# Zanue/EndoDAV

Hardware: AMD Instinct MI355X
Metric: depth frames/sec (518x518, T=8 clip) (higher is better)
Workload: dtype f32

## Files before the change

### endodav_amd/_lib.py

```python
from __future__ import annotations

import ctypes as C
import os
from typing import Optional

_HERE = os.path.dirname(os.path.abspath(__file__))
LIB_PATH = os.environ.get("EDV_LIB_PATH") or os.path.join(_HERE, "lib", "libendodav_hip.so")
ABI_VERSION = 15

LORA_TYPES = {"none": 0, "lora": 1, "dvlora": 2, "ssb": 3, "dash": 4}
ACT_NONE, ACT_GELU, ACT_RELU, ACT_SIGMOID, ACT_SIGMOID_NEG = 0, 1, 2, 3, 4


class EdvConfig(C.Structure):

    _fields_ = [
        ("abi_version", C.c_int32),
        ("embed_dim", C.c_int32),
        ("depth", C.c_int32),
        ("num_heads", C.c_int32),
        ("taps", C.c_int32 * 4),
        ("features", C.c_int32),
        ("out_channels", C.c_int32 * 4),
        ("image_h", C.c_int32),
        ("image_w", C.c_int32),
        ("num_frames", C.c_int32),
        ("pos_tokens", C.c_int32),
        ("lora_type", C.c_int32),
        ("lora_rank", C.c_int32),
        ("include_cls_token", C.c_int32),
        ("conv_head", C.c_int32),
        ("inv_sigmoid", C.c_int32),
        ("out_sigmoid", C.c_int32),
        ("temporal_lora", C.c_int32),
        ("dash_active", C.c_int32),
        ("use_clstoken", C.c_int32),
        ("residual_mask", C.c_uint32),
        ("use_bn", C.c_int32),
        ("pe_rope", C.c_int32),
    ]


_fp = C.c_void_p
_i32, _i64, _f32, _f64 = C.c_int32, C.c_int64, C.c_float, C.c_double

SIGNATURES = {
    "edv_abi_version": (C.c_int, []),
    "edv_last_error": (C.c_char_p, []),
    "edv_create": (C.c_int, [C.POINTER(EdvConfig), C.POINTER(C.c_void_p)]),
    "edv_destroy": (C.c_int, [C.c_void_p]),
    "edv_bind_param": (C.c_int, [C.c_void_p, C.c_char_p, _fp, C.POINTER(_i64), _i32]),
    "edv_prepare": (C.c_int, [C.c_void_p, C.c_void_p]),
    "edv_refresh_lora": (C.c_int, [C.c_void_p, C.c_void_p]),
    "edv_forward": (C.c_int, [C.c_void_p, _fp, _i32, _i32, _i32, _i32, C.POINTER(C.c_void_p), C.c_void_p]),
    "edv_output_shape": (C.c_int, [C.c_void_p, _i32, C.POINTER(_i32), C.POINTER(_i32)]),
    "edv_stage_copy": (C.c_int, [C.c_void_p, C.c_char_p, _fp, C.POINTER(C.c_size_t), C.c_void_p]),
    "edv_set_capture": (C.c_int, [C.c_void_p, C.c_int]),
    "edv_profile_enable": (C.c_int, [C.c_void_p, C.c_uint32]),
    "edv_set_encoder_streams": (C.c_int, [C.c_void_p, _i32]),
    "edv_set_products": (C.c_int, [C.c_void_p, _i32, C.c_void_p]),
    "edv_get_products": (C.c_int, [C.c_void_p]),
    "edv_profile_set_mask": (C.c_int, [C.c_void_p, C.c_uint32]),
    "edv_profile_work": (C.c_int, [C.c_void_p, _i32, C.POINTER(_f64), C.POINTER(_f64)]),
    "edv_profile_read": (C.c_int, [C.c_void_p, _i32, C.POINTER(_i32), C.POINTER(_f64)]),
    "edv_device_bytes": (C.c_size_t, [C.c_void_p]),
    "edv_last_launch_count": (C.c_int, [C.c_void_p]),
    "edv_layernorm": (C.c_int, [_fp, _fp, _fp, _fp, _i64, _i32, _f32, _fp, _i32, _i32, C.c_void_p]),
    "edv_gemm_workspace": (C.c_size_t, []),
    "edv_gemm_x6_planes_bytes": (C.c_size_t, [_i32, _i32]),
    "edv_gemm_x6_split": (C.c_int, [_fp, C.c_void_p, _i32, _i32, C.c_void_p]),
    "edv_gemm_x6": (C.c_int, [_fp, C.c_void_p, _fp, _i64, _i32, _i32, _fp, _i32, _fp, _fp, _fp, C.c_size_t, C.c_void_p]),
    "edv_gemm": (C.c_int, [_fp, _fp, _fp, _i64, _i32, _i32, _fp, _i32, _fp, _fp, _fp, C.c_size_t, C.c_void_p]),
    "edv_pack_geglu": (C.c_int, [_fp, _fp, _fp, _fp, _i32, _i32, C.c_void_p]),
    "edv_gemm_geglu": (C.c_int, [_fp, _fp, _fp, _fp, _i64, _i32, _i32, C.c_void_p]),
    "edv_conv3x3": (C.c_int, [_fp, _fp, _fp, _fp, _i32, _i32, _i32, _i32, _i32, _i32, _i32, _i32, _fp, _fp, C.c_void_p]),
    "edv_conv3x3_ws": (C.c_int, [_fp, _fp, _fp, _fp, _i32, _i32, _i32, _i32, _i32, _i32, _i32, _i32, _fp, _fp, _fp, C.c_size_t, C.c_void_p]),
    "edv_set_conv_impl": (C.c_int, [_i32]),
    "edv_conv3x3_dot": (C.c_int, [_fp, _fp, _fp, _fp, _i32, _i32, _i32, _i32, _i32, _i32, _i32, _i32, _fp, _fp, _i32, C.c_void_p]),
    "edv_pack_conv3x3": (C.c_int, [_fp, _fp, _i32, _i32, C.c_void_p]),
    "edv_conv_transpose": (C.c_int, [_fp, _fp, _fp, _fp, _fp, _fp, _i32, _i32, _i32, _i32, _i32, C.c_void_p]),
    "edv_attn_spatial_workspace": (C.c_size_t, [_i32, _i32, _i32]),
    "edv_attn_spatial": (C.c_int, [_fp, _fp, _i32, _i32, _i32, _fp, C.c_size_t, _fp, C.c_void_p]),
    "edv_set_train": (C.c_int, [C.c_void_p, _i32]),
    "edv_set_grad_scope": (C.c_int, [C.c_void_p, _i32, _i32, _i32, _i32]),
    "edv_set_bias_grads": (C.c_int, [C.c_void_p, _i32, _i32]),
    "edv_generation": (C.c_int, [C.c_void_p, C.POINTER(C.c_uint64)]),
    "edv_backward": (C.c_int, [C.c_void_p, C.c_uint64, _fp, C.POINTER(C.c_void_p), C.c_void_p]),
    "edv_grad_bind_flat": (C.c_int, [C.c_void_p, _i32, C.POINTER(C.c_char_p), C.POINTER(_i64), _fp, _i64, C.POINTER(_i64)]),
    "edv_grad": (C.c_int, [C.c_void_p, C.c_char_p, C.POINTER(C.c_void_p), C.POINTER(_i64)]),
    "edv_grad_copy": (C.c_int, [C.c_void_p, C.c_char_p, _fp, _i64, C.c_void_p]),
    "edv_attn_spatial_x6_workspace": (C.c_size_t, [_i32, _i32, _i32]),
    "edv_attn_spatial_x6": (C.c_int, [_fp, _fp, _i32, _i32, _i32, _fp, C.c_size_t, C.c_void_p]),
    "edv_attn_spatial_bwd_workspace": (C.c_size_t, [_i32, _i32, _i32]),
    "edv_attn_spatial_bwd": (C.c_int, [_fp, _fp, _fp, _fp, _fp, _fp, _i32, _i32, _i32, _fp, C.c_size_t, C.c_void_p]),
    "edv_layernorm_bwd": (C.c_int, [_fp, _fp, _fp, _fp, _i64, _i32, C.c_float, _i32, C.c_void_p]),
    "edv_ew_bwd": (C.c_int, [_fp, _fp, _fp, _fp, _i64, _i32, C.c_void_p]),
    "edv_geglu_bwd": (C.c_int, [_fp, _fp, _fp, _i64, _i32, C.c_void_p]),
    "edv_transpose_scale": (C.c_int, [_fp, _fp, _fp, _i32, _i32, C.c_void_p]),
    "edv_lora_grads_workspace": (C.c_size_t, [_i64, _i32, _i32, _i32]),
    "edv_lora_grads": (C.c_int, [_fp, _fp, _i64, _i32, _i32, _i32, _fp, _fp, _fp, _fp, C.c_float, _fp, _fp, C.c_size_t, _fp, _fp, _fp, _fp, C.c_void_p]),
    "edv_bilinear_bwd": (C.c_int, [_fp, _fp, _i32, _i32, _i32, _i32, _i32, _i32, _i32, C.c_void_p]),
    "edv_dot_channels_bwd": (C.c_int, [_fp, _fp, _fp, _fp, _fp, _fp, _i64, _i32, _i32, C.c_void_p]),
    "edv_conv3x3_wgrad_workspace": (C.c_size_t, [_i32, _i32, _i32, _i32, _i32]),
    "edv_conv3x3_wgrad": (C.c_int, [_fp, _fp, _fp, _i32, _i32, _i32, _i32, _i32, _fp, C.c_size_t, _i32, C.c_void_p]),
    "edv_colsum_workspace": (C.c_size_t, [_i32]),
    "edv_colsum_rows": (C.c_int, [_fp, _fp, _i64, _i32, _fp, C.c_size_t, _fp, _i32, C.c_void_p]),
    "edv_colsum_batch_workspace": (C.c_size_t, [_i32, C.POINTER(_i64), C.POINTER(_i32)]),
    "edv_colsum_batch": (C.c_int, [_i32, C.POINTER(C.c_void_p), C.POINTER(_i64), C.POINTER(_i64), C.POINTER(_i32), C.POINTER(_i32), C.POINTER(C.c_void_p),
                                   C.POINTER(C.c_void_p), C.POINTER(_i32), _fp, C.c_size_t, C.c_void_p]),
    "edv_groupnorm_bwd": (C.c_int, [_fp, _fp, _fp, _fp, _fp, _fp, _i32, _i32, _i32, _i32, _i32, C.c_void_p]),
    "edv_attn_temporal_bwd": (C.c_int, [_fp, _fp, _fp, _i32, _i32, _i32, _i32, _i32, C.c_void_p]),
    "edv_pack_conv3x3_bwd": (C.c_int, [_fp, _fp, _i32, _i32, C.c_void_p]),
    "edv_conv3x3_s2_bwd": (C.c_int, [_fp, _fp, _fp, _i32, _i32, _i32, _i32, _i32, C.c_void_p]),
    "edv_dilate2": (C.c_int, [_fp, _fp, _i32, _i32, _i32, _i32, C.c_void_p]),
    "edv_pixel_unshuffle": (C.c_int, [_fp, _fp, _i32, _i32, _i32, _i32, _i32, C.c_void_p]),
    "edv_attn_temporal": (C.c_int, [_fp, _fp, _i32, _i32, _i32, _i32, _i32, C.c_void_p]),
    "edv_groupnorm_workspace": (C.c_size_t, [_i32, _i32, _i32]),
    "edv_groupnorm": (C.c_int, [_fp, _fp, _fp, _fp, _fp, _i32, _i32, _i32, _i32, _f32, _fp, C.c_size_t, C.c_void_p]),
    "edv_geglu": (C.c_int, [_fp, _fp, _i64, _i32, C.c_void_p]),
    "edv_rope_qk": (C.c_int, [_fp, _fp, _i32, _i32, _i32, _i32, _i32, C.c_void_p]),
    "edv_trainer_loss_workspace": (C.c_size_t, [_i32, _i32, _i32]),
    "edv_trainer_loss": (C.c_int, [C.c_void_p, _i32, _i32, _i32, C.c_void_p, _fp, C.c_void_p, _fp, C.c_size_t, C.c_void_p]),
    "edv_debug_fill_lds": (C.c_int, [C.c_float, C.c_void_p]),
    "edv_bilinear": (C.c_int, [_fp, _fp, _i32, _i32, _i32, _i32, _i32, _i32, C.c_void_p]),
    "edv_dot_channels": (C.c_int, [_fp, _fp, _fp, _fp, _i64, _i32, _i32, C.c_void_p]),
    "edv_patchify": (C.c_int, [_fp, _fp, _i32, _i32, _i32, _i32, _i32, C.c_void_p]),
    "edv_bicubic_pos": (C.c_int, [_fp, _fp, _i32, _i32, _i32, _i32, _f64, _f64, C.c_void_p]),
    "edv_resize_bicubic": (C.c_int, [_fp, _fp, _i32, _i32, _i32, _i32, _i32, C.c_void_p]),
    "edv_ingest_u8": (C.c_int, [_fp, _i32, C.POINTER(_i32), _i32, _fp, _i32, _i32, _i32, _i32, C.c_void_p]),
    "edv_render_workspace": (C.c_size_t, [_i64]),
# ... 121 lines not shown
```

### endodav_amd/csrc/api.hip

```cpp
#include "../../include/endodav_hip.h"
#include <algorithm>
#include <vector>

#include "ops.hpp"

using namespace edv;

extern "C" {

int edv_layernorm(const float *x_dev, const float *w_dev, const float *b_dev, float *y_dev, int64_t rows, int32_t dim, float eps,
                  const float *pe_dev, int32_t rows_per_frame, int32_t T, void *stream) {
    return layernorm(x_dev, identity_map(), w_dev, b_dev, y_dev, identity_map(), rows, dim, eps, pe_dev, rows_per_frame, T, (hipStream_t)stream);
}

size_t edv_gemm_workspace(void) { return gemm_workspace() * sizeof(float); }
int edv_gemm(const float *A_dev, const float *W_dev, float *C_dev, int64_t M, int32_t N, int32_t K, const float *bias_dev, int32_t act,
             const float *gamma_dev, const float *R_dev, float *workspace_dev, size_t workspace_bytes, void *stream) {
    GemmDesc g;
    g.A = A_dev; g.lda = K; g.W = W_dev; g.ldw = K; g.C = C_dev; g.ldc = N; g.M = M; g.N = N; g.K = K;
    g.bias = bias_dev; g.act = act; g.gamma = gamma_dev; g.R1 = R_dev; g.ldr1 = N;
    g.ws = workspace_dev; g.ws_floats = workspace_bytes / sizeof(float);
    EDV_CHECK(act >= ACT_NONE && act <= ACT_RELU, "act must be 0, 1 or 2");
    return gemm(g, (hipStream_t)stream);
}
// ... 8 lines not shown
                const float *gamma_dev, const float *R_dev, float *workspace_dev, size_t workspace_bytes, void *stream) {
    GemmDesc g;
    g.A = A_dev; g.lda = K; g.W = reinterpret_cast<const float *>(planes_dev); g.ldw = K; g.C = C_dev; g.ldc = N; g.M = M; g.N = N; g.K = K;
    g.bias = bias_dev; g.act = act; g.gamma = gamma_dev; g.R1 = R_dev; g.ldr1 = N;
    g.ws = workspace_dev; g.ws_floats = workspace_bytes / sizeof(float);
    g.Wx6 = planes_dev;
    EDV_CHECK(act >= ACT_NONE && act <= ACT_RELU, "act must be 0, 1 or 2");
    EDV_CHECK(M > 0 && N >= 64 && K > 0 && K % 16 == 0, "edv_gemm_x6: K % 16 == 0, N >= 64");
    return gemm_x6(g, (hipStream_t)stream);
}

int edv_pack_geglu(const float *w_dev, const float *b_dev, float *wi_dev, float *bi_dev, int32_t N, int32_t K, void *stream) {
    return pack_geglu(w_dev, b_dev, wi_dev, bi_dev, N, K, (hipStream_t)stream);
}

int edv_gemm_geglu(const float *A_dev, const float *Wi_dev, const float *bi_dev, float *C_dev, int64_t M, int32_t N, int32_t K, void *stream) {
    GemmDesc g;
    g.A = A_dev; g.lda = K; g.W = Wi_dev; g.ldw = K; g.C = C_dev; g.ldc = N / 2; g.M = M; g.N = N; g.K = K;
    g.bias = bi_dev; g.geglu = 1;
    EDV_CHECK(A_dev && Wi_dev && bi_dev && C_dev && M > 0, "null operand");
    EDV_CHECK(gemm_geglu_supported(g), "edv_gemm_geglu: K % 32 == 0, N % 64 == 0, output below 4 GB");
    return gemm(g, (hipStream_t)stream);
}

static int conv3x3_impl(const float *x_dev, const float *wpacked_dev, const float *bias_dev, float *y_dev, int32_t F, int32_t H, int32_t W, int32_t Cin,
                        int32_t Cout, int32_t stride, int32_t pre_relu, int32_t post_relu, const float *R1_dev, const float *R2_dev, float *ws,
                        size_t ws_bytes, void *stream) {
    EDV_CHECK(F > 0 && H > 0 && W > 0 && Cin > 0 && Cout > 0, "empty problem");
    EDV_CHECK(stride == 1 || stride == 2, "stride must be 1 or 2");
    GemmDesc g;
    const int OH = (H - 1) / stride + 1, OW = (W - 1) / stride + 1;
    g.A = x_dev; g.W = wpacked_dev; g.ldw = 9 * Cin; g.C = y_dev; g.ldc = Cout; g.M = (long long)F * OH * OW; g.N = Cout; g.K = 9 * Cin;
    g.bias = bias_dev; g.act = post_relu ? ACT_RELU : ACT_NONE; g.R1 = R1_dev; g.ldr1 = Cout; g.R2 = R2_dev; g.ldr2 = Cout;
    g.loader = LOAD_CONV3; g.cH = H; g.cW = W; g.cC = Cin; g.cOH = OH; g.cOW = OW; g.cS = stride; g.pre_relu = pre_relu ? 1 : 0;
    g.ws = ws; g.ws_floats = ws_bytes / sizeof(float);
    return gemm(g, (hipStream_t)stream);
}

int edv_conv3x3(const float *x_dev, const float *wpacked_dev, const float *bias_dev, float *y_dev, int32_t F, int32_t H, int32_t W, int32_t Cin,
                int32_t Cout, int32_t stride, int32_t pre_relu, int32_t post_relu, const float *R1_dev, const float *R2_dev, void *stream) {
    return conv3x3_impl(x_dev, wpacked_dev, bias_dev, y_dev, F, H, W, Cin, Cout, stride, pre_relu, post_relu, R1_dev, R2_dev, nullptr, 0, stream);
}

int edv_conv3x3_ws(const float *x_dev, const float *wpacked_dev, const float *bias_dev, float *y_dev, int32_t F, int32_t H, int32_t W, int32_t Cin,
                   int32_t Cout, int32_t stride, int32_t pre_relu, int32_t post_relu, const float *R1_dev, const float *R2_dev, float *workspace_dev,
                   size_t workspace_bytes, void *stream) {
    return conv3x3_impl(x_dev, wpacked_dev, bias_dev, y_dev, F, H, W, Cin, Cout, stride, pre_relu, post_relu, R1_dev, R2_dev, workspace_dev,
                        workspace_bytes, stream);
}

int edv_set_conv_impl(int32_t mode) {
    EDV_CHECK(mode >= 0 && mode <= 2, "edv_set_conv_impl: mode 0 (automatic), 1 (never fused) or 2 (fused wherever supported)");
    set_conv_impl(mode);
    return 0;
}

int edv_conv3x3_dot(const float *x_dev, const float *wpacked_dev, const float *bias_dev, float *y_dev, int32_t F, int32_t H, int32_t W, int32_t Cin,
                    int32_t Cout, int32_t stride, int32_t pre_relu, int32_t post_relu, const float *w2_dev, const float *b2_dev, int32_t act2, void *stream) {
    EDV_CHECK(F > 0 && H > 0 && W > 0 && Cin > 0 && Cout > 0, "empty problem");
    EDV_CHECK(stride == 1 || stride == 2, "stride must be 1 or 2");
    EDV_CHECK(conv_dot_enabled(), "edv_conv3x3_dot: the fused epilogue is switched off (edv_set_conv_impl(1) or EDV_CONV_DOT=0)");
    GemmDesc g;
    const int OH = (H - 1) / stride + 1, OW = (W - 1) / stride + 1;
    g.A = x_dev; g.W = wpacked_dev; g.ldw = 9 * Cin; g.ldc = Cout; g.M = (long long)F * OH * OW; g.N = Cout; g.K = 9 * Cin;
    g.bias = bias_dev; g.act = post_relu ? ACT_RELU : ACT_NONE;
    g.loader = LOAD_CONV3; g.cH = H; g.cW = W; g.cC = Cin; g.cOH = OH; g.cOW = OW; g.cS = stride; g.pre_relu = pre_relu ? 1 : 0;
    g.w2 = w2_dev; g.b2 = b2_dev; g.act2 = act2; g.dot_out = y_dev;
    return conv_dot(g, (hipStream_t)stream);
}

int edv_pack_conv3x3(const float *w_dev, float *wpacked_dev, int32_t Cout, int32_t Cin, void *stream) {
    return pack_conv3x3(w_dev, wpacked_dev, Cout, Cin, (hipStream_t)stream);
}

int edv_conv_transpose(const float *x_dev, const float *w_dev, const float *b_dev, float *wpack_dev, float *bpack_dev, float *y_dev, int32_t F, int32_t h,
              int32_t w, int32_t C, int32_t s, void *stream) {
    EDV_CHECK(F > 0 && h > 0 && w > 0 && C > 0 && s > 0, "empty problem");
    EDV_TRY(pack_convT(w_dev, wpack_dev, b_dev, bpack_dev, C, C, s, (hipStream_t)stream));
    GemmDesc g;
    g.A = x_dev; g.lda = C; g.W = wpack_dev; g.ldw = C; g.C = y_dev; g.ldc = C; g.M = (long long)F * h * w; g.N = s * s * C; g.K = C;
    g.bias = bpack_dev; g.store = STORE_SHUFFLE; g.ps_s = s; g.ps_C = C; g.ps_h = h; g.ps_w = w;
    return gemm(g, (hipStream_t)stream);
}

size_t edv_attn_spatial_workspace(int32_t F, int32_t N, int32_t heads) { return attn_spatial_workspace(F, N, heads) * sizeof(float); }
int edv_attn_spatial(const float *qkv_dev, float *out_dev, int32_t F, int32_t N, int32_t heads, float *workspace_dev, size_t workspace_bytes,
                     float *lse_dev, void *stream) {
    return attn_spatial(qkv_dev, out_dev, F, N, heads, workspace_dev, workspace_bytes / sizeof(float), (hipStream_t)stream, lse_dev);
}
size_t edv_attn_spatial_x6_workspace(int32_t F, int32_t N, int32_t heads) { return attn_spatial_workspace(F, N, heads, true) * sizeof(float); }
int edv_attn_spatial_x6(const float *qkv_dev, float *out_dev, int32_t F, int32_t N, int32_t heads, float *workspace_dev, size_t workspace_bytes, void *stream) {
    return attn_spatial(qkv_dev, out_dev, F, N, heads, workspace_dev, workspace_bytes / sizeof(float), (hipStream_t)stream, nullptr, true);
}

size_t edv_attn_spatial_bwd_workspace(int32_t F, int32_t N, int32_t heads) { return attn_spatial_bwd_workspace(F, N, heads) * sizeof(float); }
int edv_attn_spatial_bwd(const float *qkv_dev, const float *out_dev, const float *dout_dev, const float *lse_dev, float *delta_dev, float *dqkv_dev,
                         int32_t F, int32_t N, int32_t heads, float *workspace_dev, size_t workspace_bytes, void *stream) {
    return attn_spatial_bwd(qkv_dev, out_dev, dout_dev, lse_dev, delta_dev, dqkv_dev, F, N, heads, workspace_dev, workspace_bytes / sizeof(float),
                            (hipStream_t)stream);
}
int edv_layernorm_bwd(const float *x_dev, const float *w_dev, const float *dy_dev, float *dx_dev, int64_t rows, int32_t dim, float eps, int32_t accumulate,
                      void *stream) {
    return layernorm_bwd(x_dev, identity_map(), w_dev, dy_dev, identity_map(), dx_dev, identity_map(), rows, dim, eps, accumulate != 0, (hipStream_t)stream);
}
int edv_ew_bwd(const float *d_dev, const float *src_dev, const float *add_dev, float *out_dev, int64_t n, int32_t mode, void *stream) {
    return ew_bwd(d_dev, src_dev, add_dev, out_dev, n, mode, (hipStream_t)stream);
// ... 256 lines not shown
    EDV_CHECK(row_map_from(d->a_map, &g.a_map) && row_map_from(d->c_map, &g.c_map) && row_map_from(d->r1_map, &g.r1_map) &&
                  row_map_from(d->p1_map, &g.p1_map),
              "row map: period, stride, offset >= 0 and inner 0 or 1");
    EDV_CHECK(d->act >= ACT_NONE && d->act <= ACT_RELU, "act must be 0, 1 or 2");
    EDV_CHECK(d->N > 0 && d->ldc >= d->N, "ldc must be at least N");
    EDV_CHECK(!d->R1 || d->ldr1 >= d->N, "ldr1 must be at least N");
    EDV_CHECK(!d->R2 || d->ldr2 >= d->N, "ldr2 must be at least N");
    EDV_CHECK(!d->P1 || d->ldp1 >= d->N, "ldp1 must be at least N");
    return gemm(g, (hipStream_t)stream);
}

int edv_layernorm_mapped(const float *x_dev, const int32_t *in_map, const float *w_dev, const float *b_dev, float *y_dev, const int32_t *out_map,
                         int64_t rows, int32_t dim, float eps, const float *pe_dev, int32_t rows_per_frame, int32_t T, int32_t act, int32_t accumulate,
                         void *stream) {
    RowMap im, om;
    EDV_CHECK(row_map_from(in_map, &im) && row_map_from(out_map, &om), "row map: period, stride, offset >= 0 and inner 0 or 1");
    return layernorm(x_dev, im, w_dev, b_dev, y_dev, om, rows, dim, eps, pe_dev, rows_per_frame, T, (hipStream_t)stream, act, accumulate != 0);
}

int edv_layernorm_bwd_mapped(const float *x_dev, const int32_t *x_map, const float *w_dev, const float *dy_dev, const int32_t *dy_map, float *dx_dev,
                             const int32_t *dx_map, int64_t rows, int32_t dim, float eps, int32_t accumulate, void *stream) {
    RowMap xm, gm, dm;
    EDV_CHECK(row_map_from(x_map, &xm) && row_map_from(dy_map, &gm) && row_map_from(dx_map, &dm), "row map: period, stride, offset >= 0 and inner 0 or 1");
    return layernorm_bwd(x_dev, xm, w_dev, dy_dev, gm, dx_dev, dm, rows, dim, eps, accumulate != 0, (hipStream_t)stream);
}

int edv_fold_ssb(const float *W_dev, const float *a_dev, const float *b_dev, float *out_dev, int32_t nout, int32_t nin, void *stream) {
    return fold_ssb(W_dev, a_dev, b_dev, out_dev, nout, nin, (hipStream_t)stream);
}
int edv_fold_bn(float *w_dev, const float *b_dev, const float *gamma_dev, const float *beta_dev, const float *mean_dev, const float *var_dev, float eps,
                float *bout_dev, int32_t nout, int32_t K, void *stream) {
    return fold_bn(w_dev, b_dev, gamma_dev, beta_dev, mean_dev, var_dev, eps, bout_dev, nout, K, (hipStream_t)stream);
}
int edv_fold_dash(const float *Utop_dev, const float *idx_dev, const float *Vtop_dev, float *inout_dev, int32_t nout, int32_t nin, int32_t r, void *stream) {
    return fold_dash(Utop_dev, idx_dev, Vtop_dev, inout_dev, nout, nin, r, (hipStream_t)stream);
}
int edv_col_dot(const float *P_dev, const float *Q_dev, int64_t M, int32_t N, const float *scale_dev, float *part_dev, float *out_dev, void *stream) {
    return col_dot(P_dev, Q_dev, M, N, scale_dev, part_dev, out_dev, (hipStream_t)stream);
}
int edv_ssb_prep(const float *W_dev, const float *a_dev, const float *b_dev, const float *gamma_dev, float *Wa_dev, float *gb_dev, int32_t nout,
                 int32_t nin, void *stream) {
    return ssb_prep(W_dev, a_dev, b_dev, gamma_dev, Wa_dev, gb_dev, nout, nin, (hipStream_t)stream);
}
int edv_sigmoid_bwd(const float *g_dev, const float *s_dev, float *out_dev, int64_t n, void *stream) {
    return sigmoid_bwd(g_dev, s_dev, out_dev, n, (hipStream_t)stream);
}
int edv_bilinear_add(const float *x_dev, const float *add_dev, float *y_dev, int32_t F, int32_t H, int32_t W, int32_t C, int32_t OH, int32_t OW,
                     void *stream) {
    EDV_CHECK(add_dev, "null addend");
    return bilinear(x_dev, y_dev, F, H, W, C, OH, OW, ACT_NONE, (hipStream_t)stream, add_dev);
}

int edv_split_plan(int32_t kind, int64_t tiles_or_tasks, int32_t slots, int32_t k_tiles, int64_t out[8]) {
    EDV_CHECK(out && kind >= 0 && kind <= 3 && tiles_or_tasks > 0 && tiles_or_tasks < (1ll << 31) && k_tiles > 0, "kind 0..3, a positive count below 2^31");
    if (kind == 3) {
        const TaskSplit t = plan_tasks(tiles_or_tasks, k_tiles, slots, false);
        const int64_t r[8] = {t.nsplit > 0, t.grid, t.whole_rounds, t.chunk, t.nsplit, t.leftover, t.units, (int64_t)t.pieces()};
        std::copy(r, r + 8, out);
        return 0;
    }
    const SplitPolicy &pol = kind == 0 ? gemm_dma_split_policy() : kind == 1 ? gemm_x6_split_policy() : conv_dma_split_policy();
    GemmSplit sp{};
    long long grid;
    plan_plain(tiles_or_tasks, pol, &sp, &grid);
    const bool split = plan_split(tiles_or_tasks, slots, k_tiles, pol, &sp, &grid);
    const int64_t r[8] = {split, grid, sp.whole_rounds, sp.chunk, sp.nsplit, sp.stride, sp.units, split ? (int64_t)split_ws_floats(sp, pol) : 0};
    std::copy(r, r + 8, out);
    return 0;
}

size_t edv_trainer_loss_workspace(int32_t N, int32_t H, int32_t W) { return trainer_loss_workspace(N, H, W) * sizeof(float); }
int edv_trainer_loss(const edv_trainer_loss_inputs *in, int32_t N, int32_t H, int32_t W, const edv_trainer_loss_weights *weights, float *losses_dev,
                     const edv_trainer_loss_grads *grads, float *workspace_dev, size_t workspace_bytes, void *stream) {
    EDV_CHECK(in && weights && grads, "null argument");
    TrainerLossIn a{};
    TrainerLossGrads g{};
    for (int s = 0; s < 4; ++s) {
        a.color[s] = in->color[s];
        a.disp[s] = in->disp[s];
        a.disp_h[s] = in->disp_h[s];
        a.disp_w[s] = in->disp_w[s];
        g.disp[s] = grads->disp[s];
        for (int n = 0; n < 2; ++n) {
            a.refined[s][n] = in->refined[s][n];
            a.registration[s][n] = in->registration[s][n];
            a.transform[s][n] = in->transform[s][n];
            a.position[s][n] = in->position[s][n];
            g.refined[s][n] = grads->refined[s][n];
            g.transform[s][n] = grads->transform[s][n];
        }
    }
    for (int n = 0; n < 2; ++n) {
        a.color_nb[n] = in->color_nb[n];
        a.T[n] = in->T[n];
        a.mask[n] = in->mask[n];
        g.T[n] = grads->T[n];
    }
    a.K = in->K;
    a.invK = in->invK;
    g.K = grads->K;
    g.invK = grads->invK;
    const TrainerLossW w{weights->disparity_smoothness, weights->transform_constraint, weights->transform_smoothness, weights->depth_reproj, weights->depth_flow,
                         weights->tune_temporal, weights->min_depth, weights->max_depth};
    return trainer_loss(a, N, H, W, w, losses_dev, g, workspace_dev, workspace_bytes / sizeof(float), (hipStream_t)stream);
}

size_t edv_photometric_loss_workspace(int32_t B, int32_t T, int32_t H, int32_t W) { return photometric_loss_workspace(B, T, H, W) * sizeof(float); }
// ... 11 lines not shown
```

### endodav_amd/csrc/gemm_x6.hip

```cpp
#include <algorithm>
#include <cstdio>
#include <cstdlib>
#include <type_traits>

#include "gemm_common.hpp"

#ifndef EDV_X6_STAMP
#define EDV_X6_STAMP(slot)
#endif

namespace edv {
namespace {

typedef __bf16 bf16x8 __attribute__((ext_vector_type(8)));
typedef __bf16 bf16x4 __attribute__((ext_vector_type(4)));

constexpr int XBM = 128, XBN = 128, XBK = 16;
constexpr int XPLANE = XBM * XBK * 2;
constexpr int XSTAGE = 6 * XPLANE;
constexpr int XNST = 3;
constexpr int XSLOT = XBM * XBN;
constexpr int XMAX_COUNTERS = SPLIT_MAX_COUNTERS;

__global__ __launch_bounds__(256) void split3_kernel(const float *__restrict__ w, __bf16 *__restrict__ p, long long n) {
    for (long long i = (long long)blockIdx.x * 256 + threadIdx.x; i < n; i += (long long)gridDim.x * 256) {
        const float x = w[i];
        const __bf16 h = (__bf16)x;
        const float r1 = x - (float)h;
        const __bf16 m = (__bf16)r1;
        p[i] = h;
        p[n + i] = m;
        p[2 * n + i] = (__bf16)(r1 - (float)m);
    }
}

__device__ __forceinline__ int half_pos(int r, int h) { return (h ^ ((r >> 3) & 1)) * 16; }

template <int ACT, bool SPLIT>
__global__ __launch_bounds__(256, 2) void gemm_x6_kernel(const GemmDesc g, const GemmSplit sp) {
    extern __shared__ __attribute__((aligned(16))) unsigned char smem[];
    const int tid = threadIdx.x, lane = tid & 63, wave = tid >> 6, l31 = lane & 31, lh = lane >> 5;
    const int wave_s = __builtin_amdgcn_readfirstlane(wave);
    const int wm = wave >> 1, wn = wave & 1;
    const int tiles_n = (g.N + XBN - 1) / XBN, tiles_m = (int)((g.M + XBM - 1) / XBM);
    const int G = gridDim.x;
    const int bid = xcd_remap(blockIdx.x, G);
    const int nkt = g.K / XBK;
    const __bf16 *Wp = reinterpret_cast<const __bf16 *>(g.Wx6);
    const auto rW = __builtin_amdgcn_make_buffer_rsrc(const_cast<__bf16 *>(Wp), 0, 0xffffffff, 0x00020000);
    const long long plane_bytes = (long long)g.N * g.ldw * 2;

    int fa[2], fb[2];
#pragma unroll
    for (int i = 0; i < 2; ++i) {
        const int ra = wm * 64 + i * 32 + l31, rb = wn * 64 + i * 32 + l31;
        fa[i] = ra * 32 + half_pos(ra, lh);
        fb[i] = 3 * XPLANE + rb * 32 + half_pos(rb, lh);
    }

    const int tile_l0 = sp.whole_rounds * G;
    const int run = split_run(sp, SPLIT, bid);
    long long u = split_run_begin(sp, run);
    const long long u_end = split_run_end(sp, run, u);
    int round = 0;
    for (;;) {
        int tile, kt0, kt1, lt = 0;
        float *part = nullptr;
        if (round < sp.whole_rounds) {
            tile = round * G + bid;
            kt0 = 0;
            kt1 = nkt;
            ++round;
        } else if (SPLIT && u < u_end) {
            const int t = (int)(u / nkt);
            kt0 = (int)(u - (long long)t * nkt);
            const long long left = u_end - u;
            kt1 = kt0 + left < nkt ? kt0 + (int)left : nkt;
            tile = tile_l0 + t;
            lt = t;
            if (!(kt0 == 0 && kt1 == nkt)) part = split_slot<XSLOT>(sp, run, u);
            u += kt1 - kt0;
        } else {
            break;
        }
        int tm, tn;
        {
            const int per_group = sp.group_m * tiles_n;
            const int gidx = tile / per_group, first = gidx * sp.group_m;
            const int rows = tiles_m - first < sp.group_m ? tiles_m - first : sp.group_m;
            const int r = tile - gidx * per_group;
            tn = r / rows;
            tm = first + (r - tn * rows);
        }
        const long long m0 = (long long)tm * XBM;
        const int n0 = tn * XBN;

        EDV_X6_STAMP(0);
        unsigned vw[3];
#pragma unroll
        for (int j = 0; j < 3; ++j) {
            const int id = wave * 3 + j, p = id >> 2, grp = id & 3;
            const int r = grp * 32 + (lane >> 1), pos = lane & 1;
            const int h = pos ^ ((r >> 3) & 1);
            int n = n0 + r;
            n = n < g.N ? n : g.N - 1;
            vw[j] = (unsigned)(p * plane_bytes + ((long long)n * g.ldw + h * 8) * 2);
        }
        const float *ga[2];
        int dsta[2];
#pragma unroll
        for (int j = 0; j < 2; ++j) {
            const int c = tid + 256 * j, r = c >> 2, q = c & 3;
            long long m = m0 + r;
            m = m < g.M ? m : g.M - 1;
            ga[j] = g.A + g.a_map(m) * g.lda + q * 4;
            dsta[j] = r * 32 + half_pos(r, q >> 1) + (q & 1) * 8;
        }
        auto issue_w = [&](int kt, int st) {
#pragma unroll
            for (int j = 0; j < 3; ++j) {
                const int id = wave_s * 3 + j;
// ... 132 lines not shown
#pragma unroll
                for (int j = 0; j < 2; ++j)
#pragma unroll
                    for (int r = 0; r < 16; ++r)
                        __hip_atomic_store(&part[((wave * 4 + i * 2 + j) * 16 + r) * 64 + lane], acc[i][j][r], __ATOMIC_RELAXED, __HIP_MEMORY_SCOPE_AGENT);
            const long long ub = (long long)lt * nkt;
            int g0, g1;
            store_tile = split_handoff(sp, &sp.cnt[lt], ub, nkt, reinterpret_cast<int *>(smem), tid, g0, g1);
            if (store_tile) {
#pragma unroll
                for (int i = 0; i < 2; ++i)
#pragma unroll
                    for (int j = 0; j < 2; ++j)
#pragma unroll
                        for (int r = 0; r < 16; ++r) acc[i][j][r] = 0.f;
                for (int gg = g0; gg <= g1; ++gg) {
                    const float *pp = split_piece<XSLOT>(sp.ws, sp, gg, ub) + (wave * 4 * 16) * 64 + lane;
#pragma unroll
                    for (int i = 0; i < 2; ++i)
#pragma unroll
                        for (int j = 0; j < 2; ++j) {
                            float t[16];
#pragma unroll
                            for (int r = 0; r < 16; ++r) t[r] = __hip_atomic_load(pp + ((i * 2 + j) * 16 + r) * 64, __ATOMIC_RELAXED, __HIP_MEMORY_SCOPE_AGENT);
#pragma unroll
                            for (int r = 0; r < 16; ++r) acc[i][j][r] += t[r];
                        }
                }
            }
        }
        if (store_tile) {
#pragma unroll
            for (int i = 0; i < 2; ++i)
#pragma unroll
                for (int j = 0; j < 2; ++j) {
                    EpiCols<1> c1;
                    c1.bias[0] = cols.bias[j];
                    c1.gam[0] = cols.gam[j];
                    gemm_epilogue_buf<ACT>(g, acc[i][j], c1, m0 + (wave_s >> 1) * 64 + i * 32, n0 + (wave_s & 1) * 64 + j * 32, l31, lh);
                }
        }
        EDV_X6_STAMP(3);
    }
}

template <int ACT>
int x6_slots() {
    static DeviceSlotCache cache;
    static const std::string label = "gemm_x6_kernel<" + std::to_string(ACT) + ">";
    return resident_workgroups(cache, (const void *)gemm_x6_kernel<ACT, true>, 256, XNST * XSTAGE, 2, "EDV_X6_SLOTS_PER_CU", label.c_str(),
                               (const void *)gemm_x6_kernel<ACT, false>);
}

template <int ACT>
int launch_x6(const GemmDesc &d, long long tiles, hipStream_t st) {
    const SplitPolicy &pol = gemm_x6_split_policy();
    GemmSplit sp{};
    static const int group_m = env_int("EDV_X6_GROUP_M", 8);
    sp.group_m = group_m > 0 ? group_m : 8;
    long long grid;
    plan_plain(tiles, pol, &sp, &grid);
    const int slots = x6_slots<ACT>();
    EDV_CHECK(slots > 0 && slots <= XMAX_COUNTERS, "occupancy query failed");
    if (d.ws && !gemm_plain_forced() && plan_split(tiles, slots, d.K / XBK, pol, &sp, &grid)) {
        split_bind(&sp, d.ws, pol);
        EDV_CHECK(split_ws_floats(sp, pol) <= d.ws_floats && (uintptr_t)d.ws % 16 == 0, "stream-K workspace too small (gemm_workspace)");
        EDV_LAUNCH((gemm_x6_kernel<ACT, true>), dim3((unsigned)grid), dim3(256), XNST * XSTAGE, st, d, sp);
        EDV_LAUNCH_OK();
        return 0;
    }
    EDV_LAUNCH((gemm_x6_kernel<ACT, false>), dim3((unsigned)grid), dim3(256), XNST * XSTAGE, st, d, sp);
    EDV_LAUNCH_OK();
    return 0;
}

}

const SplitPolicy &gemm_x6_split_policy() {
    static const SplitPolicy p{.min_kt = env_int("EDV_X6_SPLIT_MIN_KT", 48),
                               .min_tiles = 16, .max_rounds = 8, .widen = true, .counters = XMAX_COUNTERS, .slot_floats = XSLOT, .whole_rounds = true};
    return p;
}

size_t gemm_x6_planes_bytes(int N, int K) { return (size_t)3 * N * K * 2; }

int gemm_x6_split(const float *W, void *planes, int N, int K, hipStream_t st) {
    EDV_CHECK(W && planes && N > 0 && K > 0, "null argument");
    const long long n = (long long)N * K;
    EDV_LAUNCH(split3_kernel, dim3((unsigned)std::min<long long>((n + 255) / 256, 2048)), dim3(256), 0, st, W, reinterpret_cast<__bf16 *>(planes), n);
    EDV_LAUNCH_OK();
    return 0;
}

bool gemm_x6_supported(const GemmDesc &d) {
    const int ek = epilogue_kind(d);
    if (d.a_map.period != 0) return false;
    if (!(d.Wx6 && d.loader == LOAD_DENSE && ek >= 1 && ek <= 3 && d.K % XBK == 0 && d.lda % 4 == 0 && d.ldw == d.K && d.M > 0 && d.N >= 64)) return false;
    if (!((long long)3 * d.N * d.K * 2 < (1ll << 32) - (1 << 20))) return false;
    const long long ld = std::max(std::max(d.ldc, d.R1 ? d.ldr1 : 0), d.R2 ? d.ldr2 : 0);
    return (long long)(d.M + XBM) * ld * 4 < (1ll << 32) - 4096;
}

int gemm_x6(const GemmDesc &d, hipStream_t st) {
    EDV_CHECK(d.A && d.Wx6 && d.C, "null operand");
    EDV_CHECK(gemm_x6_supported(d), "bf16x6 GEMM: dense A, planes of a [N, K] weight, K % 16 == 0, identity row maps, outputs below 4 GB");
    EDV_CHECK(d.lda >= d.K, "leading dimension");
    EDV_CHECK(((uintptr_t)d.A % 16 == 0) && ((uintptr_t)d.Wx6 % 16 == 0), "A / planes must be 16-byte aligned");
    const long long tiles = ((d.M + XBM - 1) / XBM) * (long long)((d.N + XBN - 1) / XBN);
    EDV_CHECK(tiles > 0 && tiles < (1ll << 31), "bad grid");
    switch (epilogue_kind(d)) {
        case 1: return launch_x6<ACT_NONE>(d, tiles, st);
        case 2: return launch_x6<ACT_GELU>(d, tiles, st);
        default: return launch_x6<ACT_RELU>(d, tiles, st);
    }
}

}
```

### endodav_amd/csrc/ops.hpp

```cpp
#pragma once
#include "common.hpp"
#include "streamk_plan.hpp"

namespace edv {

enum { ACT_NONE = 0, ACT_GELU = 1, ACT_RELU = 2, ACT_SIGMOID = 3, ACT_SIGMOID_NEG = 4 };
enum { LOAD_DENSE = 0, LOAD_CONV3 = 1 };
enum { STORE_ROWS = 0, STORE_SHUFFLE = 1 };

struct GemmDesc {
    const float *A = nullptr;
    int lda = 0;
    RowMap a_map{0, 0, 0};
    const float *W = nullptr;
    int ldw = 0;
    float *C = nullptr;
    int ldc = 0;
    RowMap c_map{0, 0, 0};
    long long M = 0;
    int N = 0, K = 0;
    const float *bias = nullptr;
    int act = ACT_NONE;
    const float *gamma = nullptr;
    const float *R1 = nullptr;
    int ldr1 = 0;
    RowMap r1_map{0, 0, 0};
    const float *R2 = nullptr;
    int ldr2 = 0;
    const float *P1 = nullptr;
    int ldp1 = 0;
    RowMap p1_map{0, 0, 0};
    int loader = LOAD_DENSE;
    int cH = 0, cW = 0, cC = 0, cOH = 0, cOW = 0, cS = 1, pre_relu = 0;
    int store = STORE_ROWS;
    int geglu = 0;
    int ps_s = 0, ps_C = 0, ps_h = 0, ps_w = 0;
    float *ws = nullptr;
    size_t ws_floats = 0;
    const void *Wx6 = nullptr;
    const float *w2 = nullptr, *b2 = nullptr;
    float *dot_out = nullptr;
    int act2 = ACT_NONE;
};
int gemm(const GemmDesc &d, hipStream_t st);
size_t gemm_x6_planes_bytes(int N, int K);
int gemm_x6_split(const float *W, void *planes, int N, int K, hipStream_t st);
bool gemm_x6_supported(const GemmDesc &d);
int gemm_x6(const GemmDesc &d, hipStream_t st);
size_t gemm_workspace();
size_t gemm_counter_bytes();
bool gemm_dma_supported(const GemmDesc &d);
bool gemm_geglu_supported(const GemmDesc &d);
int pack_geglu(const float *w, const float *b, float *wi, float *bi, int N, int K, hipStream_t st);
int gemm_dma(const GemmDesc &d, hipStream_t st);
bool conv_dma_supported(const GemmDesc &d);
int conv_dma(const GemmDesc &d, hipStream_t st);
bool conv_dot_supported(const GemmDesc &d);
int conv_dot(const GemmDesc &d, hipStream_t st);
bool conv_halo_supported(const GemmDesc &d);
bool conv_halo_wanted(const GemmDesc &d);
int conv_halo(const GemmDesc &d, hipStream_t st);
void set_conv_impl(int mode);
int conv_impl();
bool conv_dot_enabled();
const SplitPolicy &gemm_dma_split_policy();
const SplitPolicy &gemm_x6_split_policy();
const SplitPolicy &conv_dma_split_policy();
const char *gemm_kernel_name(const GemmDesc &d);

size_t attn_spatial_workspace(int F, int N, int heads, bool x6 = false);
int attn_spatial(const float *qkv, float *out, int F, int N, int heads, float *ws, size_t ws_floats, hipStream_t st, float *lse = nullptr, bool x6 = false);
size_t attn_spatial_bwd_workspace(int F, int N, int heads);
int attn_spatial_bwd(const float *qkv, const float *out, const float *dout, const float *lse, float *delta, float *dqkv, int F, int N, int heads, float *ws,
                     size_t ws_floats, hipStream_t st);
int attn_temporal(const float *qkv, float *out, int B, int T, int P, int C, int heads, hipStream_t st);
int geglu(const float *x, float *y, long long M, int inner, hipStream_t st);
int rope_qk(float *qkv, const float *table, int B, int T, int P, int C, bool transpose, hipStream_t st);

int layernorm(const float *x, RowMap in_map, const float *w, const float *b, float *y, RowMap out_map, long long rows, int dim,
              float eps, const float *pe, int rows_per_frame, int T, hipStream_t st, int act = ACT_NONE, bool accumulate = false);
size_t groupnorm_workspace(int F, int P, int C);
int groupnorm(const float *x, const float *w, const float *b, float *y, float *stats, int F, int P, int C, int groups, float eps, hipStream_t st,
              float *part = nullptr, size_t part_floats = 0);

int patchify(const float *x, float *cols, int F, int H, int W, int ih, int iw, hipStream_t st, int ld = 588)  ;
int bilinear(const float *x, float *y, int F, int H, int W, int C, int OH, int OW, int act, hipStream_t st, const float *add = nullptr);
int dot_channels(const float *x, const float *w, const float *b, float *y, long long M, int C, int act, hipStream_t st);
int cls_rows(const float *cls, const float *pos, float *tokens, int F, int ntok, int D, hipStream_t st);
int sigmoid_inplace(float *x, long long n, hipStream_t st);
int resize_bicubic(const float *x, float *y, int NP, int H, int W, int OH, int OW, hipStream_t st);
int ingest_u8(const uint8_t *src, int src_frames, const int32_t *slots_host, int n, float *out, int H, int W, int OH, int OW, hipStream_t st);
size_t stitch_workspace();
int stitch_fit(const float *disp, int ih, int iw, const float *tail, int fh, int fw, float *st, void *ws, size_t ws_bytes, hipStream_t stream);
int stitch_apply(const float *disp, int ih, int iw, const float *st, float *tail, float *out_new, int fh, int fw, hipStream_t stream);
size_t metrics_workspace(long long n, int h, int w);
int masked_median(const float *x, const float *gate, long long count, float lo, float hi, double *out, void *ws, size_t ws_bytes, hipStream_t stream);
int metrics_pred(const float *disp, const float *gt, float *pred, long long n, int h, int w, double min_depth, double max_depth, int align, float factor, float cap,
                 double *scal, void *ws, size_t ws_bytes, hipStream_t stream);
int metrics_errors(const float *pred, const float *gt, long long n, int h, int w, float cap, double *out, void *ws, size_t ws_bytes, hipStream_t stream);
int metrics_temporal(const float *pred, const float *gt, long long n, int h, int w, float cap, const double *mats, double *out, float *warp, void *ws,
                     size_t ws_bytes, hipStream_t stream);
size_t render_workspace(long long n);
int render_range(const float *x, long long n, int h, int w, int mode, long long rank_lo, long long rank_hi, float *range, void *ws, size_t ws_bytes, hipStream_t stream);
int render_colorize(const float *x, long long n, int h, int w, const float *range, int range_stride, float eps, int clip, const uint8_t *lut, const uint8_t *beside,
                    uint8_t *out, hipStream_t stream);
struct CloudSel {
    const float *x;
    long long n;
    int h, w, step, mode;
    float lo, span, gain, near_z, far_z;
    const uint8_t *mask;
    long long mask_stride;
};
int cloud_tile_pixels();
size_t cloud_workspace(long long n, int h, int w, int step);
int cloud_count(const CloudSel &s, long long *offsets, void *ws, size_t ws_bytes, hipStream_t stream);
int cloud_scatter(const CloudSel &s, const double *cams, int cam_stride, const uint8_t *frames, const long long *offsets, const void *ws, size_t ws_bytes,
                  float *points, uint8_t *colors, long long capacity, hipStream_t stream);
struct TsdfVol {
    float *tsdf, *weight, *color;
// ... 109 lines not shown
```

### endodav_amd/csrc/streamk_plan.hpp

```cpp
#pragma once
#include <cstddef>

namespace edv {

struct GemmSplit {
    int whole_rounds, chunk, nsplit, stride;
    long long units;
    float *ws;
    int *cnt;
    int group_m = 1;
};

struct SplitPolicy {
    int min_kt;
    int min_tiles;
    int max_rounds;
    bool widen;
    int counters;
    int slot_floats;
    bool whole_rounds;
    int deep_kt = 0, idle_factor = 0;
};

inline void plan_plain(long long tiles, const SplitPolicy &p, GemmSplit *sp, long long *grid) {
    sp->whole_rounds = p.whole_rounds ? 1 : 0;
    sp->chunk = 1;
    sp->nsplit = 0;
    sp->stride = 1;
    sp->units = 0;
    *grid = tiles;
}

inline bool plan_split(long long tiles, int slots, int nkt, const SplitPolicy &p, GemmSplit *sp, long long *grid) {
    if (slots <= 0 || tiles <= p.min_tiles || nkt < p.min_kt) return false;
    const long long left = p.whole_rounds ? tiles % slots : tiles;
    if (p.whole_rounds ? !(left > 0 && tiles < (long long)p.max_rounds * slots)
                       : !(tiles <= slots && tiles <= p.counters && (nkt >= p.deep_kt || tiles * p.idle_factor <= slots)))
        return false;
    sp->whole_rounds = p.whole_rounds ? (int)(tiles / slots) : 0;
    long long split_tiles = left;
    const long long chunk_min = (nkt + 3) / 4;
    if (p.widen && sp->whole_rounds > 0 && (left * nkt + slots - 1) / slots < chunk_min && left + slots <= p.counters) {
        --sp->whole_rounds;
        split_tiles += slots;
    }
    sp->units = split_tiles * nkt;
    long long chunk = (sp->units + slots - 1) / slots;
    chunk = chunk > chunk_min ? chunk : chunk_min;
    sp->chunk = (int)chunk;
    sp->nsplit = (int)((sp->units + chunk - 1) / chunk);
    *grid = sp->whole_rounds ? slots : (sp->nsplit > 0 ? sp->nsplit : 1);
    sp->stride = (int)(*grid / sp->nsplit) > 0 ? (int)(*grid / sp->nsplit) : 1;
    return true;
}

inline size_t split_ws_floats(const GemmSplit &sp, const SplitPolicy &p) { return (size_t)p.counters + (size_t)sp.nsplit * 2 * p.slot_floats; }

inline void split_bind(GemmSplit *sp, float *ws, const SplitPolicy &p) {
    sp->cnt = reinterpret_cast<int *>(ws);
    sp->ws = ws + p.counters;
}

struct TaskSplit {
    int grid, whole_rounds, chunk, leftover, nsplit;
    long long units;
    size_t pieces() const { return (size_t)nsplit * 2; }
};
inline TaskSplit plan_tasks(long long ntasks, int ntiles, int slots, bool plain) {
    TaskSplit p;
    if (plain || slots <= 0) {
        p.grid = (int)ntasks; p.whole_rounds = 1; p.leftover = 0; p.units = 0; p.chunk = 1; p.nsplit = 0;
        return p;
    }
    p.whole_rounds = (int)(ntasks / slots);
    p.leftover = (int)(ntasks - (long long)p.whole_rounds * slots);
    p.units = (long long)p.leftover * ntiles;
    p.chunk = p.units ? (int)((p.units + slots - 1) / slots) : 1;
    p.nsplit = (int)((p.units + p.chunk - 1) / p.chunk);
    p.grid = p.whole_rounds ? slots : p.nsplit;
    return p;
}

}
```

### include/endodav_hip.h

```cpp
#ifndef ENDODAV_HIP_H
#define ENDODAV_HIP_H

#include <stddef.h>
#include <stdint.h>

#ifdef __cplusplus
extern "C" {
#endif

#define EDV_ABI_VERSION 15

enum edv_lora_type { EDV_LORA_NONE = 0, EDV_LORA_LORA = 1, EDV_LORA_DVLORA = 2, EDV_LORA_SSB = 3, EDV_LORA_DASH = 4 };

typedef struct edv_config {
    int32_t abi_version;
    int32_t embed_dim;
    int32_t depth;
    int32_t num_heads;
    int32_t taps[4];
    int32_t features;
    int32_t out_channels[4];
    int32_t image_h, image_w;
    int32_t num_frames;
    int32_t pos_tokens;
// ... 231 lines not shown
int edv_attn_temporal_bwd(const float *qkv_dev, const float *dout_dev, float *dqkv_dev, int32_t B, int32_t T, int32_t P, int32_t C, int32_t heads,
                          void *stream);
int edv_pack_conv3x3_bwd(const float *w_dev, float *wpacked_dev, int32_t Cout, int32_t Cin, void *stream);
int edv_conv3x3_s2_bwd(const float *dy_dev, const float *wpacked_dev, float *dx_dev, int32_t F, int32_t H, int32_t W, int32_t Cin, int32_t Cout,
                       void *stream);
int edv_dilate2(const float *dy_dev, float *z_dev, int32_t F, int32_t H, int32_t W, int32_t C, void *stream);
int edv_pixel_unshuffle(const float *dy_dev, float *A_dev, int32_t F, int32_t h, int32_t w, int32_t C, int32_t s, void *stream);

typedef struct edv_gemm_desc_t {
    const float *A;
    int32_t lda;
    int32_t a_map[4];
    const float *W;
    int32_t ldw;
    float *C;
    int32_t ldc;
    int32_t c_map[4];
    int64_t M;
    int32_t N, K;
    const float *bias;
    int32_t act;
    const float *gamma;
    const float *R1;
    int32_t ldr1;
    int32_t r1_map[4];
    const float *R2;
    int32_t ldr2;
    const float *P1;
    int32_t ldp1;
    int32_t p1_map[4];
    float *workspace;
    size_t workspace_bytes;
    const void *x6_planes;
} edv_gemm_desc_t;
int edv_gemm_desc(const edv_gemm_desc_t *d, void *stream);
int edv_layernorm_mapped(const float *x_dev, const int32_t *in_map, const float *w_dev, const float *b_dev, float *y_dev, const int32_t *out_map,
                         int64_t rows, int32_t dim, float eps, const float *pe_dev, int32_t rows_per_frame, int32_t T, int32_t act, int32_t accumulate,
                         void *stream);
int edv_layernorm_bwd_mapped(const float *x_dev, const int32_t *x_map, const float *w_dev, const float *dy_dev, const int32_t *dy_map, float *dx_dev,
                             const int32_t *dx_map, int64_t rows, int32_t dim, float eps, int32_t accumulate, void *stream);
int edv_fold_ssb(const float *W_dev, const float *a_dev, const float *b_dev, float *out_dev, int32_t nout, int32_t nin, void *stream);
int edv_fold_bn(float *w_dev, const float *b_dev, const float *gamma_dev, const float *beta_dev, const float *mean_dev, const float *var_dev, float eps,
                float *bout_dev, int32_t nout, int32_t K, void *stream);
int edv_fold_dash(const float *Utop_dev, const float *idx_dev, const float *Vtop_dev, float *inout_dev, int32_t nout, int32_t nin, int32_t r, void *stream);
int edv_col_dot(const float *P_dev, const float *Q_dev, int64_t M, int32_t N, const float *scale_dev, float *part_dev, float *out_dev, void *stream);
int edv_ssb_prep(const float *W_dev, const float *a_dev, const float *b_dev, const float *gamma_dev, float *Wa_dev, float *gb_dev, int32_t nout,
                 int32_t nin, void *stream);
int edv_sigmoid_bwd(const float *g_dev, const float *s_dev, float *out_dev, int64_t n, void *stream);
int edv_bilinear_add(const float *x_dev, const float *add_dev, float *y_dev, int32_t F, int32_t H, int32_t W, int32_t C, int32_t OH, int32_t OW,
                     void *stream);

int edv_split_plan(int32_t kind, int64_t tiles_or_tasks, int32_t slots, int32_t k_tiles, int64_t out[8]);

#ifdef __cplusplus
}
#endif
#endif
```

Baseline: 1126.

## Add remainder stream-K plan for x6 GEMM splitting only leftover tiles across CUs

Adds a new stream-K planning mode for the bf16 x6 GEMM. Whole tiles fill complete rounds over the CU count, and only the leftover tiles (tiles mod CUs) are split along K into chunked runs. Those split runs are placed at the front of the grid and the whole tiles are remapped per XCD. This targets the tail-wave imbalance when the tile count is slightly above a multiple of the CU count, at the cost of workspace reductions and extra fixup work for the split tiles. It is enabled by default (mode 1, by policy) and adds an API to control it.

Measured after the change: 1160, median of 6. +3.0%, better.

```diff
diff --git a/endodav_amd/_lib.py b/endodav_amd/_lib.py
--- a/endodav_amd/_lib.py
+++ b/endodav_amd/_lib.py
@@ -76,6 +76,7 @@
     "edv_conv3x3": (C.c_int, [_fp, _fp, _fp, _fp, _i32, _i32, _i32, _i32, _i32, _i32, _i32, _i32, _fp, _fp, C.c_void_p]),
     "edv_conv3x3_ws": (C.c_int, [_fp, _fp, _fp, _fp, _i32, _i32, _i32, _i32, _i32, _i32, _i32, _i32, _fp, _fp, _fp, C.c_size_t, C.c_void_p]),
     "edv_set_conv_impl": (C.c_int, [_i32]),
+    "edv_set_x6_remainder": (C.c_int, [_i32, _i32]),
     "edv_conv3x3_dot": (C.c_int, [_fp, _fp, _fp, _fp, _i32, _i32, _i32, _i32, _i32, _i32, _i32, _i32, _fp, _fp, _i32, C.c_void_p]),
     "edv_pack_conv3x3": (C.c_int, [_fp, _fp, _i32, _i32, C.c_void_p]),
     "edv_conv_transpose": (C.c_int, [_fp, _fp, _fp, _fp, _fp, _fp, _i32, _i32, _i32, _i32, _i32, C.c_void_p]),
diff --git a/endodav_amd/csrc/api.hip b/endodav_amd/csrc/api.hip
--- a/endodav_amd/csrc/api.hip
+++ b/endodav_amd/csrc/api.hip
@@ -84,6 +84,12 @@
 int edv_set_conv_impl(int32_t mode) {
     EDV_CHECK(mode >= 0 && mode <= 2, "edv_set_conv_impl: mode 0 (automatic), 1 (never fused) or 2 (fused wherever supported)");
     set_conv_impl(mode);
+    return 0;
+}
+
+int edv_set_x6_remainder(int32_t mode, int32_t cus) {
+    EDV_CHECK(mode >= 0 && mode <= 2 && cus >= 0, "edv_set_x6_remainder: mode 0 (off), 1 (by policy) or 2 (wherever supported); cus 0 = the device's count");
+    set_x6_remainder(mode, cus);
     return 0;
 }
 
@@ -446,7 +452,26 @@
 }
 
 int edv_split_plan(int32_t kind, int64_t tiles_or_tasks, int32_t slots, int32_t k_tiles, int64_t out[8]) {
-    EDV_CHECK(out && kind >= 0 && kind <= 3 && tiles_or_tasks > 0 && tiles_or_tasks < (1ll << 31) && k_tiles > 0, "kind 0..3, a positive count below 2^31");
+    if (kind == 5) {
+        EDV_CHECK(out && slots > 0 && k_tiles >= 0 && k_tiles <= slots && tiles_or_tasks >= k_tiles && tiles_or_tasks < slots, "kind 5: nsplit <= block < grid");
+        std::fill(out, out + 8, 0);
+        out[0] = front_whole_tile((int)tiles_or_tasks, slots, k_tiles);
+        return 0;
+    }
+    EDV_CHECK(out && kind >= 0 && kind <= 4 && tiles_or_tasks > 0 && tiles_or_tasks < (1ll << 31) && k_tiles > 0, "kind 0..5, a positive count below 2^31");
+    if (kind == 4) {
+        const int wgs = (int)out[0], mode = (int)out[1];
+        EDV_CHECK(slots > 0 && wgs > 0 && wgs <= 64 && (mode == 1 || mode == 2), "kind 4: out[0] = workgroups per CU, out[1] = mode 1 or 2");
+        const SplitPolicy &pol = gemm_x6_split_policy();
+        GemmSplit sp{};
+        long long grid;
+        plan_plain(tiles_or_tasks, pol, &sp, &grid);
+        const bool rem = gemm_x6_plan(tiles_or_tasks, k_tiles, slots * wgs, slots, wgs, mode, &sp, &grid) == 2;
+        const int64_t r[8] = {1, grid, sp.first_split, sp.chunk, sp.nsplit, tiles_or_tasks - sp.first_split, sp.units, (int64_t)split_ws_floats(sp, pol)};
+        std::fill(out, out + 8, 0);
+        if (rem) std::copy(r, r + 8, out);
+        return 0;
+    }
     if (kind == 3) {
         const TaskSplit t = plan_tasks(tiles_or_tasks, k_tiles, slots, false);
         const int64_t r[8] = {t.nsplit > 0, t.grid, t.whole_rounds, t.chunk, t.nsplit, t.leftover, t.units, (int64_t)t.pieces()};
diff --git a/endodav_amd/csrc/gemm_x6.hip b/endodav_amd/csrc/gemm_x6.hip
--- a/endodav_amd/csrc/gemm_x6.hip
+++ b/endodav_amd/csrc/gemm_x6.hip
@@ -44,7 +44,8 @@
     const int wm = wave >> 1, wn = wave & 1;
     const int tiles_n = (g.N + XBN - 1) / XBN, tiles_m = (int)((g.M + XBM - 1) / XBM);
     const int G = gridDim.x;
-    const int bid = xcd_remap(blockIdx.x, G);
+    const bool front = SPLIT && sp.front != 0;
+    const int bid = front ? front_whole_tile(blockIdx.x, G, sp.nsplit) : xcd_remap(blockIdx.x, G);
     const int nkt = g.K / XBK;
     const __bf16 *Wp = reinterpret_cast<const __bf16 *>(g.Wx6);
     const auto rW = __builtin_amdgcn_make_buffer_rsrc(const_cast<__bf16 *>(Wp), 0, 0xffffffff, 0x00020000);
@@ -58,15 +59,16 @@
         fb[i] = 3 * XPLANE + rb * 32 + half_pos(rb, lh);
     }
 
-    const int tile_l0 = sp.whole_rounds * G;
-    const int run = split_run(sp, SPLIT, bid);
+    const int tile_l0 = front ? sp.first_split : sp.whole_rounds * G;
+    const int run = front ? ((int)blockIdx.x < sp.nsplit ? (int)blockIdx.x : -1) : split_run(sp, SPLIT, bid);
+    const int whole_rounds = front ? (run < 0 ? 1 : 0) : sp.whole_rounds;
     long long u = split_run_begin(sp, run);
     const long long u_end = split_run_end(sp, run, u);
     int round = 0;
     for (;;) {
         int tile, kt0, kt1, lt = 0;
         float *part = nullptr;
-        if (round < sp.whole_rounds) {
+        if (round < whole_rounds) {
             tile = round * G + bid;
             kt0 = 0;
             kt1 = nkt;
@@ -305,6 +307,17 @@
                                (const void *)gemm_x6_kernel<ACT, false>);
 }
 
+std::atomic<int> g_x6_rem_mode{1}, g_x6_rem_cus{0};
+
+int device_cus() {
+    static DeviceSlotCache cache;
+    return cache.get([] {
+        int dev = 0, cus = 0;
+        if (hipGetDevice(&dev) != hipSuccess || hipDeviceGetAttribute(&cus, hipDeviceAttributeMultiprocessorCount, dev) != hipSuccess) return 0;
+        return cus;
+    });
+}
+
 template <int ACT>
 int launch_x6(const GemmDesc &d, long long tiles, hipStream_t st) {
     const SplitPolicy &pol = gemm_x6_split_policy();
@@ -315,7 +328,10 @@
     plan_plain(tiles, pol, &sp, &grid);
     const int slots = x6_slots<ACT>();
     EDV_CHECK(slots > 0 && slots <= XMAX_COUNTERS, "occupancy query failed");
-    if (d.ws && !gemm_plain_forced() && plan_split(tiles, slots, d.K / XBK, pol, &sp, &grid)) {
+    const int dev_cus = device_cus(), set_cus = g_x6_rem_cus.load(std::memory_order_relaxed);
+    EDV_CHECK(dev_cus > 0, "device query failed");
+    if (d.ws && !gemm_plain_forced() &&
+        gemm_x6_plan(tiles, d.K / XBK, slots, set_cus > 0 && set_cus < dev_cus ? set_cus : dev_cus, slots / dev_cus, g_x6_rem_mode.load(std::memory_order_relaxed), &sp, &grid)) {
         split_bind(&sp, d.ws, pol);
         EDV_CHECK(split_ws_floats(sp, pol) <= d.ws_floats && (uintptr_t)d.ws % 16 == 0, "stream-K workspace too small (gemm_workspace)");
         EDV_LAUNCH((gemm_x6_kernel<ACT, true>), dim3((unsigned)grid), dim3(256), XNST * XSTAGE, st, d, sp);
@@ -333,6 +349,21 @@
     static const SplitPolicy p{.min_kt = env_int("EDV_X6_SPLIT_MIN_KT", 48),
                                .min_tiles = 16, .max_rounds = 8, .widen = true, .counters = XMAX_COUNTERS, .slot_floats = XSLOT, .whole_rounds = true};
     return p;
+}
+
+const RemainderPolicy &gemm_x6_remainder_policy() {
+    static const RemainderPolicy p{.left_div = 16, .run_div = 6, .min_run = 3, .runs_per_cu = 2, .counters = XMAX_COUNTERS};
+    return p;
+}
+
+int gemm_x6_plan(long long tiles, int nkt, int slots, int cus, int wgs_per_cu, int mode, GemmSplit *sp, long long *grid) {
+    if (mode != 0 && plan_remainder(tiles, nkt, cus, wgs_per_cu, mode == 2, gemm_x6_remainder_policy(), sp, grid)) return 2;
+    return plan_split(tiles, slots, nkt, gemm_x6_split_policy(), sp, grid) ? 1 : 0;
+}
+
+void set_x6_remainder(int mode, int cus) {
+    g_x6_rem_mode.store(mode < 0 || mode > 2 ? 1 : mode, std::memory_order_relaxed);
+    g_x6_rem_cus.store(cus > 0 ? cus : 0, std::memory_order_relaxed);
 }
 
 size_t gemm_x6_planes_bytes(int N, int K) { return (size_t)3 * N * K * 2; }
diff --git a/endodav_amd/csrc/ops.hpp b/endodav_amd/csrc/ops.hpp
--- a/endodav_amd/csrc/ops.hpp
+++ b/endodav_amd/csrc/ops.hpp
@@ -66,6 +66,9 @@
 const SplitPolicy &gemm_dma_split_policy();
 const SplitPolicy &gemm_x6_split_policy();
 const SplitPolicy &conv_dma_split_policy();
+const RemainderPolicy &gemm_x6_remainder_policy();
+int gemm_x6_plan(long long tiles, int nkt, int slots, int cus, int wgs_per_cu, int mode, GemmSplit *sp, long long *grid);
+void set_x6_remainder(int mode, int cus);
 const char *gemm_kernel_name(const GemmDesc &d);
 
 size_t attn_spatial_workspace(int F, int N, int heads, bool x6 = false);
diff --git a/endodav_amd/csrc/streamk_plan.hpp b/endodav_amd/csrc/streamk_plan.hpp
--- a/endodav_amd/csrc/streamk_plan.hpp
+++ b/endodav_amd/csrc/streamk_plan.hpp
@@ -9,6 +9,7 @@
     float *ws;
     int *cnt;
     int group_m = 1;
+    int front = 0, first_split = 0;
 };
 
 struct SplitPolicy {
@@ -28,6 +29,8 @@
     sp->nsplit = 0;
     sp->stride = 1;
     sp->units = 0;
+    sp->front = 0;
+    sp->first_split = 0;
     *grid = tiles;
 }
 
@@ -52,6 +55,44 @@
     *grid = sp->whole_rounds ? slots : (sp->nsplit > 0 ? sp->nsplit : 1);
     sp->stride = (int)(*grid / sp->nsplit) > 0 ? (int)(*grid / sp->nsplit) : 1;
     return true;
+}
+
+struct RemainderPolicy {
+    int left_div;
+    int run_div;
+    int min_run;
+    int runs_per_cu;
+    int counters;
+};
+
+inline bool plan_remainder(long long tiles, int nkt, int cus, int wgs_per_cu, bool everywhere, const RemainderPolicy &p, GemmSplit *sp, long long *grid) {
+    if (cus <= 0 || wgs_per_cu <= 0 || tiles < cus || nkt < p.min_run) return false;
+    const long long left = tiles % cus;
+    if (left == 0 || left > p.counters || (!everywhere && left * p.left_div > cus)) return false;
+    const long long units = left * nkt;
+    const long long cap = (long long)cus * (wgs_per_cu < p.runs_per_cu ? wgs_per_cu : p.runs_per_cu);
+    long long chunk = nkt / p.run_div > p.min_run ? nkt / p.run_div : p.min_run;
+    if ((units + cap - 1) / cap > chunk) chunk = (units + cap - 1) / cap;
+    const long long nsplit = (units + chunk - 1) / chunk;
+    if (!everywhere && nsplit + (tiles - left) > (long long)cus * wgs_per_cu) return false;
+    sp->whole_rounds = 1;
+    sp->chunk = (int)chunk;
+    sp->nsplit = (int)nsplit;
+    sp->stride = 1;
+    sp->units = units;
+    sp->front = 1;
+    sp->first_split = (int)(tiles - left);
+    *grid = sp->nsplit + (tiles - left);
+    return true;
+}
+
+#ifdef __HIPCC__
+__host__ __device__
+#endif
+inline int front_whole_tile(int b, int G, int nsplit) {
+    const int x = b & 7;
+    const int before = ((G >> 3) * x + (x < (G & 7) ? x : (G & 7))) - ((nsplit >> 3) * x + (x < (nsplit & 7) ? x : (nsplit & 7)));
+    return before + (b >> 3) - ((nsplit + 7 - x) >> 3);
 }
 
 inline size_t split_ws_floats(const GemmSplit &sp, const SplitPolicy &p) { return (size_t)p.counters + (size_t)sp.nsplit * 2 * p.slot_floats; }
diff --git a/include/endodav_hip.h b/include/endodav_hip.h
--- a/include/endodav_hip.h
+++ b/include/endodav_hip.h
@@ -307,6 +307,8 @@
 
 int edv_split_plan(int32_t kind, int64_t tiles_or_tasks, int32_t slots, int32_t k_tiles, int64_t out[8]);
 
+int edv_set_x6_remainder(int32_t mode, int32_t cus);
+
 #ifdef __cplusplus
 }
 #endif
```
